# YannisLamp/crypto-recommendation

Measured on AMD Instinct MI355X. Metric: point hash+assign ops/sec at d=128, N=10M, K=256; 1/2/4/8 MI355X, higher is better.
Workload: dtype fp32 points; split-f16 MFMA scores (f32 accumulate); tuples, bucket IDs and cluster IDs bit-exact (x87-exact hashing, certified argmin); distances: certified f32, <= 2^-20 relative to the reference's fp64 (north star: 1e-5; the context's default LSHKM_DIST_CERTIFIED mode), LSHKM_DIST_EXACT for the r; 1 GPU; C3 Lloyd K=256 + C2 LSH L=5 k=4 hashing, N=10000000 per GPU, d=128; N_per_gpu=10000000, N_total=10000000, d=128, K=256, L=5, k=4, nb=100000, parallelism=dp1 (row shards)

## Files before the change

crypto-recommendation_amd/csrc/fused_hi.hip:

```cpp
#include "fused_impl.h"

namespace lshkm {

__host__ __device__ constexpr int fh_lds_bytes(int Kpad, bool hash) {
    return 16 + Kpad * FU_RS * 2 + Kpad * 4 + (hash ? 2 * 32 * FU_RS * 2 + FP_HC_BYTES : 0);
}
static_assert(fh_lds_bytes(FH_KMAX, true) <= 160 * 1024, "hi-only LDS image exceeds 160 KiB");
constexpr double FH_A = 130.0 * 0x1p-23;

constexpr int FH_WAVES_MPFAST = 12;
constexpr int FH_FAST_WAVES = 8;
template <bool HASH, bool MP, int MET, bool FAST = false>
__host__ __device__ constexpr int fh_waves() {
    return HASH && MP ? 12 : (MP && FAST ? FH_WAVES_MPFAST : (FAST && !MP ? FH_FAST_WAVES : 8));
}

__device__ inline int cosine_halves_finish(double sh0, double sl0, double ts0, double sh, double sl, double ts,
                                           double xa, double nbv, double& v) {
    const double mb = 2.0 * sqrt(__dmul_rn(xa, nbv)) * (1.0 + 0x1p-40);
    const double tsum = __dadd_rn(ts0, ts);
    if (!(tsum >= 0x1p-790)) return 2;
    IpAcc ip;
    const double t = __dadd_rn(sh0, sh);
    const double bb = __dsub_rn(t, sh0);
    const double e = __dadd_rn(__dsub_rn(sh0, __dsub_rn(t, bb)), __dsub_rn(sh, bb));
    ip.sh = t;
    ip.sl = __dadd_rn(__dadd_rn(sl0, sl), e);
    ip.ts = __dadd_rn(tsum * (1.0 + 0x1p-47), 0x1p-37 * mb);
    ip.mx = mb;
    double q, qr;
    const int st = ip.quot_status(__dmul_rn(sqrt(xa), sqrt(nbv)), q, qr);
    if (st == 0) v = __dsub_rn(1.0, q);
    return st;
}

__device__ inline int cosine_winner_halves(const float (&xf)[64], const double* __restrict__ crow_h, double nbv, int h,
                                           double& v) {
    double xa = 0.0;
#pragma unroll
    for (int s = 0; s < 8; s++) {
        if (h == 0) {
#pragma unroll
            for (int j = 0; j < 8; j++) {
                const double xj = (double)xf[8 * s + j];
                xa = __dadd_rn(xa, __dmul_rn(xj, xj));
            }
        }
        xa = take_from_lower(xa);
        if (h == 1) {
#pragma unroll
            for (int j = 0; j < 8; j++) {
                const double xj = (double)xf[8 * s + j];
                xa = __dadd_rn(xa, __dmul_rn(xj, xj));
            }
        }
        xa = take_from_upper(xa);
    }
    double sh = 0.0, sl = 0.0, ts = 0.0;
    double off = 0.0;
    double2 cb[4];
#pragma unroll
    for (int j = 0; j < 4; j++) cb[j] = *reinterpret_cast<const double2*>(crow_h + 2 * j);
#pragma unroll
    for (int s = 0; s < 8; s++) {
        double cv[8];
#pragma unroll
        for (int j = 0; j < 4; j++) { cv[2 * j] = cb[j].x; cv[2 * j + 1] = cb[j].y; }
        if (s + 1 < 8) {
#pragma unroll
            for (int j = 0; j < 4; j++) cb[j] = *reinterpret_cast<const double2*>(crow_h + 16 * (s + 1) + 2 * j);
        }
#pragma unroll
        for (int j = 0; j < 8; j++) {
            const double pj = __dmul_rn((double)xf[8 * s + j], cv[j]);
            const double t = __dadd_rn(sh, pj);
            const double bb = __dsub_rn(t, sh);
            const double e = __dadd_rn(__dsub_rn(sh, __dsub_rn(t, bb)), __dsub_rn(pj, bb));
            sh = t;
            sl = __dadd_rn(sl, e);
            ts = __dadd_rn(ts, fabs(__dadd_rn(t, off)));
        }
        const double other = swap_halves(sh, h);
        if (h == 1) ts = __dadd_rn(ts, 8.0 * fabs(__dsub_rn(other, off)));
        off = other;
    }
    const double sh0 = swap_halves(sh, h), sl0 = swap_halves(sl, h), ts0 = swap_halves(ts, h);
    if (h == 0) return 2;
    return cosine_halves_finish(sh0, sl0, ts0, sh, sl, ts, xa, nbv, v);
}

__device__ inline int cosine_winner_halves_x64(const FusedArgs& a, int64_t rowc, const double* __restrict__ crow_h,
                                               double nbv, int h, double& v) {
    double2 xn[4], xnn[4];
    load_x64_step(a, rowc, 0, h, xn);
    load_x64_step(a, rowc, 1, h, xnn);
    double sh = 0.0, sl = 0.0, ts = 0.0;
    double off = 0.0;
    double2 cb[4];
#pragma unroll
    for (int j = 0; j < 4; j++) cb[j] = *reinterpret_cast<const double2*>(crow_h + 2 * j);
#pragma unroll 1
    for (int s = 0; s < 8; s++) {
        double xv[8], cv[8];
#pragma unroll
        for (int j = 0; j < 4; j++) {
            xv[2 * j] = xn[j].x; xv[2 * j + 1] = xn[j].y;
            cv[2 * j] = cb[j].x; cv[2 * j + 1] = cb[j].y;
            xn[j] = xnn[j];
        }
        if (s + 2 < 8) load_x64_step(a, rowc, s + 2, h, xnn);
        if (s + 1 < 8) {
#pragma unroll
            for (int j = 0; j < 4; j++) cb[j] = *reinterpret_cast<const double2*>(crow_h + 16 * (s + 1) + 2 * j);
        }
#pragma unroll
        for (int j = 0; j < 8; j++) {
            const double pj = __dmul_rn(xv[j], cv[j]);
            const double t = __dadd_rn(sh, pj);
            const double bb = __dsub_rn(t, sh);
            const double e = __dadd_rn(__dsub_rn(sh, __dsub_rn(t, bb)), __dsub_rn(pj, bb));
            sh = t;
            sl = __dadd_rn(sl, e);
            ts = __dadd_rn(ts, fabs(__dadd_rn(t, off)));
        }
        const double other = swap_halves(sh, h);
        if (h == 1) ts = __dadd_rn(ts, 8.0 * fabs(__dsub_rn(other, off)));
        off = other;
    }
    const double sh0 = swap_halves(sh, h), sl0 = swap_halves(sl, h), ts0 = swap_halves(ts, h);
    if (h == 0) return 2;
    return cosine_halves_finish(sh0, sl0, ts0, sh, sl, ts, a.xn2[rowc], nbv, v);
}

constexpr int FH_GATH_STEP = 32 * 16 * 8;
constexpr int FH_GATH_WAVE = 2 * FH_GATH_STEP;
__host__ __device__ constexpr int fh_gath_off(int Kpad, bool hash) { return (fh_lds_bytes(Kpad, hash) + 255) & ~255; }
static_assert(fh_gath_off(FH_GATH_KMAX, true) + 8 * FH_GATH_WAVE <= 160 * 1024, "gather ring exceeds 160 KiB");

__device__ inline void glds16(const void* gsrc, uint32_t lds_dst) {
    unsigned keep;
    asm volatile("s_mov_b32 %0, m0\n\ts_mov_b32 m0, %2\n\ts_nop 0\n\tglobal_load_lds_dwordx4 %1, off\n\ts_mov_b32 m0, %0"
                 : "=&s"(keep) : "v"(gsrc), "s"(lds_dst) : "memory");
}

#ifndef LSHKM_ROWPF
#define LSHKM_ROWPF 3
#endif
constexpr int FH_ROWPF = LSHKM_ROWPF;
constexpr int FH_ROWPF_KMAX = 256;
constexpr int FH_ROWPF_WAVE = 32 * 64 * 4;
__host__ __device__ constexpr int fh_rowpf_off(int Kpad, bool hash) { return (fh_lds_bytes(Kpad, hash) + 255) & ~255; }
static_assert(fh_rowpf_off(FH_ROWPF_KMAX, true) + FH_FAST_WAVES * FH_ROWPF_WAVE <= 160 * 1024,
              "row prefetch buffers exceed 160 KiB");
static_assert(FH_ROWPF_KMAX <= FH_GATH_KMAX, "the FAST single-pass form runs where the gather ring would (fused.hip)");

__device__ inline void glds16s(const void* sbase, uint32_t voff, uint32_t lds_base, int lds_off) {
    unsigned keep;
    asm volatile("s_mov_b32 %0, m0\n\ts_add_u32 m0, %3, %4\n\ts_nop 0\n\tglobal_load_lds_dwordx4 %1, %2\n\ts_mov_b32 m0, %0"
                 : "=&s"(keep) : "v"(voff), "s"(sbase), "s"(lds_base), "n"(lds_off) : "memory", "scc");
}

template <bool HASH, bool MP = false, int MET = 0, int NIMG = 1, bool GATH = false, int ROWS = 0, bool FAST = false,
          int PF = 0>
__global__ __launch_bounds__((64 * fh_waves<HASH, MP, MET, FAST>()), 1) void fused_hi_kernel(FusedArgs a) {
    constexpr int FH_WAVES = fh_waves<HASH, MP, MET, FAST>();
    constexpr int FH_THREADS = 64 * FH_WAVES;
    static_assert(NIMG == 1 || (!MP && MET == 0), "two-image form: euclidean, single launch");
    static_assert(!GATH || (!MP && MET == 0 && NIMG == 1 && FH_WAVES == 8), "gather ring: euclidean single pass");
    static_assert(ROWS == 0 || (!HASH && !MP && NIMG == 1), "general rows: Lloyd without hashing, one pass");
    static_assert(!(GATH && ROWS == 2), "fp64 rows re-read x in the chain: register loads of the winner rows");
    static_assert(!FAST || (MET == 0 && ROWS != 2 && NIMG == 1 && !GATH), "fast distance: euclidean, fp32 rows");
    static_assert(PF == 0 || (FAST && !MP && ROWS == 0 && FH_WAVES == FH_FAST_WAVES), "row prefetch: the FAST single-pass form");
    constexpr bool PFR = (PF & 1) != 0, PFL = (PF & 2) != 0;
    extern __shared__ __attribute__((aligned(16))) char smem[];
    const int Kpad = a.Kpad;
    const bool fastd = FAST || a.fast_dist != 0;
    const int KI = NIMG == 2 ? FH_KMAX : Kpad;
    int* lcount = reinterpret_cast<int*>(smem);
    _Float16* lch = reinterpret_cast<_Float16*>(smem + 16);
    float* lcn = reinterpret_cast<float*>(lch + KI * FU_RS);
    _Float16* lvh = reinterpret_cast<_Float16*>(lcn + KI);
    _Float16* lvl = lvh + 32 * FU_RS;
    float* lpn0 = reinterpret_cast<float*>(lvl + 32 * FU_RS);
    float* lv10 = lpn0 + 32;
    float* lt0 = lv10 + 32;
    int32_t* lr0 = reinterpret_cast<int32_t*>(lt0 + 32);

    auto load_image = [&](int img) {
        const int r0 = img * KI, nr = NIMG == 2 && img == 1 ? Kpad - FH_KMAX : KI;
        constexpr int FH_CU = 8;
        for (int e0 = 0; e0 < nr * 16; e0 += FH_THREADS * FH_CU) {
            float4 v[FH_CU];
#pragma unroll
            for (int u = 0; u < FH_CU; u++) {
                const int e = e0 + u * FH_THREADS + (int)threadIdx.x < nr * 16 ? e0 + u * FH_THREADS + (int)threadIdx.x : 0;
                v[u] = *reinterpret_cast<const float4*>(a.Ch + (size_t)(r0 + (e >> 4)) * FU_D + (e & 15) * 8);
            }
#pragma unroll
            for (int u = 0; u < FH_CU; u++) {
                const int e = e0 + u * FH_THREADS + (int)threadIdx.x < nr * 16 ? e0 + u * FH_THREADS + (int)threadIdx.x : 0;
                *reinterpret_cast<float4*>(lch + (e >> 4) * FU_RS + (e & 15) * 8) = v[u];
            }
        }
        for (int e = threadIdx.x; e < nr; e += FH_THREADS) lcn[e] = a.cnh[r0 + e];
    };
    load_image(0);
    if (threadIdx.x < 3) lcount[threadIdx.x] = 0;
    int32_t* ambig_seg = a.ambig + (int64_t)blockIdx.x * a.seg_rows;
    unsigned long long* hfix_seg = a.hfix + (int64_t)blockIdx.x * a.seg_rows;
    unsigned long long* cfix_seg = a.cfix ? a.cfix + (int64_t)blockIdx.x * a.seg_rows : nullptr;
    if (HASH) {
        hash_stage_images<FH_THREADS>(a.Vh, a.Vl, lvh, lvl);
        if (threadIdx.x < 32) {
            const int f = threadIdx.x;
            const bool on = f < a.LK;
            float P = 0.f, Q = 0.f;
            if (on) hash_window<MET == 0>(a.pnorm[f], a.v1[f], MET == 0 ? a.tv[f] : 0.f, a.w, P, Q);
            lpn0[f] = P;
            lv10[f] = Q;
            lt0[f] = on && MET == 0 ? a.tv[f] : 0.f;
            lr0[f] = on && MET == 0 ? a.rv[f] : 0;
        }
    }
    __syncthreads();

    const int lane = threadIdx.x & 63;
    const int wave = PF != 0 ? __builtin_amdgcn_readfirstlane((int)(threadIdx.x >> 6)) : (int)(threadIdx.x >> 6);
    const int col = lane & 31, h = lane >> 5;
    const float cmaxf = a.cbound[3], crf = a.cbound[4], chf = a.cbound[5], cnf = a.cbound[6];
    const bool c_ok = __float_as_uint(a.cbound[2]) == 0u;
    const _Float16* my_h = lch + col * FU_RS + 8 * h;
    const int ntile32 = Kpad >> 5;
    const int64_t ntiles = (a.N + 31) >> 5;
    const double Ec = (0x1p-24 + FH_A) * (double)cnf + 0x1p-41 * (double)cmaxf * (double)cmaxf + 0x1p-18 * (double)cnf;

    const int64_t tstride = (int64_t)gridDim.x * FH_WAVES, tfirst = (int64_t)blockIdx.x * FH_WAVES;
    const int64_t nround = NIMG == 2 && ntiles > tfirst ? (ntiles - tfirst + tstride - 1) / tstride : 0;
    int64_t rd = 0;
    auto load_row = [&](int64_t tl, float (&dst)[64]) {
        const int64_t rr = tl * 32 + col, rc = rr < a.N ? rr : a.N - 1;
        if constexpr (ROWS != 0) load_row_gen<ROWS>(a, rc, h, dst);
        else load_row_b(a.X + rc * FU_D + 8 * h, dst);
    };
    auto load_half = [&](int64_t tl, int hf, float* dst) {
        const int64_t rr = tl * 32 + col, rc = rr < a.N ? rr : a.N - 1;
        const float* xr = a.X + rc * FU_D + 64 * hf + 8 * h;
#pragma unroll
        for (int s = 0; s < 4; s++) {
            const float4 p0 = *reinterpret_cast<const float4*>(xr + 16 * s);
            const float4 p1 = *reinterpret_cast<const float4*>(xr + 16 * s + 4);
            dst[8 * s + 0] = p0.x; dst[8 * s + 1] = p0.y; dst[8 * s + 2] = p0.z; dst[8 * s + 3] = p0.w;
            dst[8 * s + 4] = p1.x; dst[8 * s + 5] = p1.y; dst[8 * s + 6] = p1.z; dst[8 * s + 7] = p1.w;
        }
    };
    uint32_t pfbase = 0;
    if constexpr (PFL)
        pfbase = (uint32_t)__builtin_amdgcn_readfirstlane(
            (int)((uint32_t)(uintptr_t)(smem + fh_rowpf_off(Kpad, HASH)) + (uint32_t)wave * FH_ROWPF_WAVE));
    auto pf_dma = [&](int64_t tl) {
        const int64_t tls = ((int64_t)__builtin_amdgcn_readfirstlane((int)(tl >> 32)) << 32) |
                            (uint32_t)__builtin_amdgcn_readfirstlane((int)tl);
        const int64_t left = a.N - 1 - tls * 32;
        const int pmax = left < 31 ? (int)left : 31;
        const float* xt = a.X + tls * 32 * FU_D;
        if (pmax == 31) {
            const uint32_t w0 = (uint32_t)((lane >> 4) * (FU_D * 4) + 16 * ((lane & 15) ^ (lane >> 4)));
#pragma unroll
            for (int u = 0; u < 8; u++) glds16s(xt + u * 4 * FU_D, w0 ^ (uint32_t)(64 * (u & 3)), pfbase, u * 1024);
        } else {
#pragma unroll
            for (int u = 0; u < 8; u++) {
                const int p = 4 * u + (lane >> 4), pc = p < pmax ? p : pmax;
                glds16s(xt, (uint32_t)(pc * (FU_D * 4) + 16 * ((lane & 15) ^ (p & 15))), pfbase, u * 1024);
            }
        }
    };
    float xn[32];
    auto pf_next = [&](int64_t tl) {
        if constexpr (PF != 0) {
            if (tl + tstride < ntiles) {
                if constexpr (PFL) {
                    __builtin_amdgcn_s_waitcnt(0xC07F);
                    asm volatile("" ::: "memory");
                    pf_dma(tl + tstride);
                }
                if constexpr (PFR) load_half(tl + tstride, 1, xn);
            } else if constexpr (PFR) {
#pragma unroll
                for (int j = 0; j < 32; j++) xn[j] = 0.f;
            }
        }
    };
    if constexpr (PF != 0) {
        if (tfirst + wave < ntiles) {
            if constexpr (PFL) pf_dma(tfirst + wave);
            if constexpr (PFR) load_half(tfirst + wave, 1, xn);
            if constexpr (PFL) {
                __builtin_amdgcn_s_waitcnt(0x0F70);
                asm volatile("" ::: "memory");
            }
        }
    }
    PT_DECL
    for (int64_t tile = tfirst + wave; NIMG == 2 ? rd < nround : tile < ntiles; tile += tstride, rd++) {
        const int64_t row = tile * 32 + col;
        const bool valid = row < a.N;
        float xf[64];
        if constexpr (PF == 0) {
            load_row(tile, xf);
        } else {
            if constexpr (PFL) {
                if constexpr (!PFR) {
                    load_half(tile, 1, xf + 32);
                    asm volatile("" ::: "memory");
                }
                __builtin_amdgcn_s_waitcnt(PFR ? 0x4F70 : 0x0F78);
                asm volatile("" ::: "memory");
                const char* pb = smem + fh_rowpf_off(Kpad, HASH) + wave * FH_ROWPF_WAVE + col * 256;
#pragma unroll
                for (int c = 0; c < 8; c++) {
                    const float4 v = *reinterpret_cast<const float4*>(pb + 16 * ((4 * (c >> 1) + 2 * h + (c & 1)) ^ (col & 15)));
                    xf[4 * c] = v.x; xf[4 * c + 1] = v.y; xf[4 * c + 2] = v.z; xf[4 * c + 3] = v.w;
                }
            } else {
                load_half(tile, 0, xf);
            }
            if constexpr (PFR) {
#pragma unroll
                for (int j = 0; j < 32; j++) xf[32 + j] = xn[j];
            }
        }
        half8 bh[8];
        float2v n2a = {0.f, 0.f}, n2b = {0.f, 0.f}, r2 = {0.f, 0.f};
        double xn2, nx, nxr, nxh;
        bool x_ok;
        auto finish_norms = [&]() {
            float xn2f = (n2a.x + n2a.y) + (n2b.x + n2b.y);
            float xr2f = r2.x + r2.y;
            xn2f += __shfl_xor(xn2f, 32);
            xr2f += __shfl_xor(xr2f, 32);
            xn2 = (double)xn2f * (1.0 + 0x1p-16);
            nx = sqrt(xn2);
            nxr = sqrt((double)xr2f * (1.0 + 0x1p-16)) + 0x1p-100;
            if (ROWS == 2) nxr += 0x1p-24 * nx * (1.0 + 0x1p-20);
            nxh = nx + nxr;
            x_ok = xn2f <= FU_RANGE * FU_RANGE;
        };
        const bool hash_here = HASH;
        if (!hash_here) {
#pragma unroll
            for (int s = 0; s < 8; s++) {
                half8 unused;
                split_norm_step<false>(xf + 8 * s, bh[s], unused, n2a, n2b, r2);
            }
            pf_next(tile);
            finish_norms();
        }

        if (hash_here) {
            uint32_t fmask = 0;
            float acc_hi[16];
            {
                const _Float16* vh_row = lvh + col * FU_RS + 8 * h;
                const _Float16* vl_row = lvl + col * FU_RS + 8 * h;
                floatx16 tot;
#pragma unroll
                for (int s = 0; s < 8; s++) {
                    half8 bl;
                    split_norm_step<true>(xf + 8 * s, bh[s], bl, n2a, n2b, r2);
                    const floatx16 acc = hash_tile_step(s, vh_row, vl_row, bh[s], bl);
                    if (s == 0) {
                        tot = acc;
                    } else {
#pragma unroll
                        for (int r = 0; r < 16; r += 2) {
                            const float2v t2 = {tot[r], tot[r + 1]}, a2 = {acc[r], acc[r + 1]};
                            const float2v u2 = t2 + a2;
                            tot[r] = u2.x;
                            tot[r + 1] = u2.y;
                        }
                    }
                }
#pragma unroll
                for (int r = 0; r < 16; r++) acc_hi[r] = tot[r];
            }
            finish_norms();
            const float iw = MET == 1 ? 1.f : 1.0f / a.w;
            const float nxf = (float)nx * (1.f + 0x1p-20f);
            int hc = 0;
            asm volatile("" : "+v"(hc));
            const float* lt = lt0 + hc;
            const float* lP = lpn0 + hc;
            const float* lQ = lv10 + hc;
            const int32_t* lr = lr0 + hc;
            if (!x_ok && valid) fmask = (a.LK >= 32 ? 0xFFFFFFFFu : (1u << a.LK) - 1u);
#pragma unroll
            for (int g = 0; g < 4; g++) {
                const int l = 2 * g + h;
                if (l >= a.L || !valid) continue;
                const int64_t o = row * a.L + l;
                if constexpr (MET == 1) {
                    int gv = 0;
#pragma unroll
                    for (int q = 0; q < 4; q++) {
                        const int f = 4 * l + q;
                        int bit;
                        if (!certify_sign_f32(acc_hi[4 * g + q], nxf, lP[f], lQ[f], bit)) fmask |= 1u << f;
                        gv = (gv << 1) | bit;
                    }
                    if (a.phi) a.phi[o] = gv;
                    if (a.bucket) a.bucket[o] = gv;
                    continue;
                }
                int32_t hv[4];
#pragma unroll
                for (int q = 0; q < 4; q++) {
                    const int f = 4 * l + q;
                    if (!certify_floor_f32(acc_hi[4 * g + q], lt[f], iw, nxf, lP[f], lQ[f], hv[q])) fmask |= 1u << f;
                }
                if (a.tuples) *reinterpret_cast<int4*>(a.tuples + o * 4) = make_int4(hv[0], hv[1], hv[2], hv[3]);
                uint32_t hn = 0;
#pragma unroll
                for (int q = 0; q < 4; q++) hn += phi_term_small(hv[q], lr[4 * l + q]);
                const uint32_t ph = phi_final(hn);
                if (a.phi) a.phi[o] = (int32_t)ph;
                if (a.bucket) a.bucket[o] = bucket_fast(ph, a.bdiv);
            }
            fmask |= __shfl_xor(fmask, 32);
            const unsigned long long fb = __ballot(fmask != 0u && h == 1);
            if (fb) {
                const int leader = __builtin_ctzll(fb);
                int base = 0;
                if (lane == leader) base = atomicAdd(lcount + 1, __popcll(fb));
                base = __shfl(base, leader);
                if (fmask != 0u && h == 1)
                    hfix_seg[base + __popcll(fb & ((1ull << lane) - 1ull))] = ((unsigned long long)row << 32) | fmask;
            }
        }

        if (HASH) pf_next(tile);
        PT_MARK(0)
        const double E = (nxh * (double)crf + nxr * (double)cmaxf + FH_A * nxh * (double)chf + 0x1p-41 * xn2 +
                          0x1p-18 * nx * (double)cmaxf + (MET == 1 ? 0x1p-43 * nx : 0.0) + Ec) * (1.0 + 0x1p-20) +
                         1e-30;
        float m1 = -__builtin_inff(), m2 = -__builtin_inff();
        int t1 = 0;
        if (MP && !HASH && !a.pass_first) {
            const float4 st = a.part[tile * 64 + lane];
            m1 = st.x; m2 = st.y; t1 = __float_as_int(st.z);
        }
        const int tg0 = MP ? a.t0 : 0;
        __builtin_amdgcn_s_setprio(MFMA_PRIO);
        const int ntile_run = ntile32;
        auto run_tiles = [&](int ntl, int tgo) {
#pragma unroll 1
            for (int t = 0; t < ntl; t++) {
                const float m1_prev = m1;
                floatx16 acc;
                const float* cn_t = lcn + t * 32 + 4 * h;
#pragma unroll
                for (int g = 0; g < 4; g++) {
                    const float4 cn = *reinterpret_cast<const float4*>(cn_t + 8 * g);
                    acc[4 * g] = cn.x; acc[4 * g + 1] = cn.y; acc[4 * g + 2] = cn.z; acc[4 * g + 3] = cn.w;
                }
                const _Float16* arow = my_h + t * 32 * FU_RS;
#pragma unroll
                for (int s = 0; s < 8; s++) {
                    const half8 ah = *reinterpret_cast<const half8*>(arow + 16 * s);
                    acc = __builtin_amdgcn_mfma_f32_32x32x16_f16(ah, bh[s], acc, 0, 0, 0);
                }
                float sv[16];
#pragma unroll
                for (int r = 0; r < 16; r++) sv[r] = acc[r];
                tile_epilogue(sv, m1, m2);
                t1 = m1 != m1_prev ? t + tgo : t1;
            }
        };
        if (NIMG == 1) {
            run_tiles(ntile_run, tg0);
        } else {
            const int i0 = (int)(rd & 1);
            const int nA = FH_KMAX / 32, nB = (Kpad - FH_KMAX) / 32;
            run_tiles(i0 == 0 ? nA : nB, i0 * nA);
            __syncthreads();
            load_image(1 - i0);
            __syncthreads();
            run_tiles(i0 == 0 ? nB : nA, (1 - i0) * nA);
        }
        __builtin_amdgcn_s_setprio(0);
        PT_MARK(1)
        if (MP && (HASH || !a.pass_last)) {
            a.part[tile * 64 + lane] = make_float4(m1, m2, __int_as_float(t1), 0.f);
            continue;
        }
        const uint32_t l1 = __float_as_uint(m1) & 0xFu;
        const int i1 = t1 * 32 + 8 * (int)(l1 >> 2) + 4 * h + (int)(l1 & 3u);
        const float om1 = __shfl_xor(m1, 32), om2 = __shfl_xor(m2, 32);
        const int oi1 = __shfl_xor(i1, 32);
        const float M2 = fmaxf(fmaxf(m2, om2), fminf(m1, om1));
        const int I1 = (om1 > m1 || (om1 == m1 && oi1 < i1)) ? oi1 : i1;
        const float M1 = fmaxf(m1, om1);
        const double* crow = a.C64 + (size_t)I1 * FU_D + 8 * h;
        const char* gsrc[4];
        uint32_t gbase = 0;
        const bool g32 = GATH && a.C32 != nullptr && (__float_as_uint(a.cbound[7]) & 1u) == 0u;
        const int gstep = g32 ? 64 : 128;
        if (GATH && !fastd) {
            gbase = (uint32_t)__builtin_amdgcn_readfirstlane(
                (int)((uint32_t)(uintptr_t)(smem + fh_gath_off(Kpad, HASH)) + (uint32_t)wave * FH_GATH_WAVE));
            if (g32) {
#pragma unroll
                for (int u = 0; u < 2; u++) {
                    const int p = 16 * u + (lane >> 2);
                    const int Ip = __shfl(I1, p);
                    gsrc[u] = reinterpret_cast<const char*>(a.C32 + (size_t)Ip * FU_D + 4 * ((lane & 3) ^ ((p >> 2) & 3)));
                }
                gsrc[2] = gsrc[3] = gsrc[0];
#pragma unroll
                for (int s0 = 0; s0 < 2; s0++)
#pragma unroll
                    for (int u = 0; u < 2; u++) glds16(gsrc[u] + gstep * s0, gbase + s0 * FH_GATH_STEP + u * 1024);
            } else {
#pragma unroll
                for (int u = 0; u < 4; u++) {
                    const int p = 8 * u + (lane >> 3);
                    const int Ip = __shfl(I1, p);
                    gsrc[u] = reinterpret_cast<const char*>(a.C64 + (size_t)Ip * FU_D + 2 * ((lane & 7) ^ ((p >> 1) & 7)));
                }
#pragma unroll
                for (int s0 = 0; s0 < 2; s0++)
#pragma unroll
                    for (int u = 0; u < 4; u++) glds16(gsrc[u] + gstep * s0, gbase + s0 * FH_GATH_STEP + u * 1024);
            }
        }
        double2 gnext[4];
        float4 gnext32[2];
        auto gread = [&](int st) {
            const char* ring = smem + fh_gath_off(Kpad, HASH) + wave * FH_GATH_WAVE + (st & 1) * FH_GATH_STEP;
            if (g32) {
#pragma unroll
                for (int j = 0; j < 2; j++)
                    gnext32[j] = *reinterpret_cast<const float4*>(ring + (col >> 4) * 1024 + (col & 15) * 64 +
                                                                  16 * ((2 * h + j) ^ ((col >> 2) & 3)));
            } else {
#pragma unroll
                for (int j = 0; j < 4; j++)
                    gnext[j] = *reinterpret_cast<const double2*>(ring + col * 128 + 16 * ((4 * h + j) ^ ((col >> 1) & 7)));
            }
        };
        auto wait_step = [&]() {
            if (g32) __builtin_amdgcn_s_waitcnt(0x0F72);
            else __builtin_amdgcn_s_waitcnt(0x0F74);
        };
        auto ring_advance = [&](int s) {
            if (s + 2 < 8) {
                __builtin_amdgcn_s_waitcnt(0xC07F);
                asm volatile("" ::: "memory");
                if (g32) {
#pragma unroll
                    for (int u = 0; u < 2; u++) glds16(gsrc[u] + gstep * (s + 2), gbase + (s & 1) * FH_GATH_STEP + u * 1024);
                } else {
#pragma unroll
                    for (int u = 0; u < 4; u++) glds16(gsrc[u] + gstep * (s + 2), gbase + (s & 1) * FH_GATH_STEP + u * 1024);
                }
            }
            if (s + 1 < 8) {
                if (s + 2 < 8) wait_step();
                else __builtin_amdgcn_s_waitcnt(0x0F70);
                asm volatile("" ::: "memory");
                gread(s + 1);
            }
        };
        constexpr int XD = 4;
        double2 xring[XD][4];
        const int64_t rowc = row < a.N ? row : a.N - 1;
        if constexpr (ROWS == 2 && MET == 0) {
#pragma unroll
            for (int st = 0; st < XD; st++) load_x64_step(a, rowc, st, h, xring[st]);
        }
        double2 cbuf[4];
        if (MET == 0 && !GATH && !fastd) {
#pragma unroll
            for (int j = 0; j < 4; j++) cbuf[j] = *reinterpret_cast<const double2*>(crow + 2 * j);
        }
        const bool cert = x_ok && c_ok && ((double)M2 < (double)M1 - 2.0 * E);

        bool dok = true;
        double fdist = 0.0;
        if constexpr (MET == 0) {
            if (fastd) {
                const float* c32 = a.C32 + (size_t)I1 * FU_D + 8 * h;
                float2v q[4] = {};
                float4 cc[16];
                if constexpr (PF != 0) {
#pragma unroll
                    for (int s = 0; s < 8; s++) {
                        cc[2 * s] = *reinterpret_cast<const float4*>(c32 + 16 * s);
                        cc[2 * s + 1] = *reinterpret_cast<const float4*>(c32 + 16 * s + 4);
                    }
                    __builtin_amdgcn_sched_barrier(0);
                }
#pragma unroll
                for (int s = 0; s < 8; s++) {
                    float4 c0, c1;
                    if constexpr (PF != 0) {
                        c0 = cc[2 * s]; c1 = cc[2 * s + 1];
                    } else {
                        c0 = *reinterpret_cast<const float4*>(c32 + 16 * s);
                        c1 = *reinterpret_cast<const float4*>(c32 + 16 * s + 4);
                    }
                    const float2v cv[4] = {{c0.x, c0.y}, {c0.z, c0.w}, {c1.x, c1.y}, {c1.z, c1.w}};
#pragma unroll
                    for (int j = 0; j < 4; j++) {
                        const float2v xv = {xf[8 * s + 2 * j], xf[8 * s + 2 * j + 1]};
                        const float2v dv = xv - cv[j];
                        q[j] = __builtin_elementwise_fma(dv, dv, q[j]);
                    }
                }
                float t = ((q[0].x + q[0].y) + (q[1].x + q[1].y)) + ((q[2].x + q[2].y) + (q[3].x + q[3].y));
                t = t + swap_halves_f(t, h);
                const double S = (double)t, R = (double)a.rn32[I1];
                const double B = 14.2 * 0x1p-24 * S + 2.02 * R * sqrt(S) + 2.02 * R * R + 0x1p-100;
                dok = B <= 0x1p-19 * S;
                fdist = sqrt(S);
            }
        }
        const bool amb = valid && !(cert && dok);
        const unsigned long long amask = __ballot(amb && h == 1);
        if (amb && h == 1) {
            int base = 0;
            const int leader = __builtin_ctzll(amask);
            if (lane == leader) base = atomicAdd(lcount, __popcll(amask));
            base = __shfl(base, leader);
            ambig_seg[base + __popcll(amask & ((1ull << lane) - 1ull))] = (int32_t)row;
        }
        if constexpr (MET == 1) {
            bool fix = false;
            if (valid && cert) {
                double v = 0.0;
                int st;
                if constexpr (ROWS == 2) st = cosine_winner_halves_x64(a, row, a.C64 + (size_t)I1 * FU_D + 8 * h, a.nbv[I1], h, v);
                else st = cosine_winner_halves(xf, a.C64 + (size_t)I1 * FU_D + 8 * h, a.nbv[I1], h, v);
                if (h == 1) {
                    a.assign[row] = I1;
                    if (st == 0) a.dist[row] = v;
                    else fix = true;
                }
            }
            const unsigned long long fb = __ballot(fix);
            if (fb) {
                const int leader = __builtin_ctzll(fb);
                int base = 0;
                if (lane == leader) base = atomicAdd(lcount + 2, __popcll(fb));
                base = __shfl(base, leader);
                if (fix) cfix_seg[base + __popcll(fb & ((1ull << lane) - 1ull))] = (unsigned long long)row;
            }
        } else if (fastd) {
            if (h == 1 && valid && cert && dok) {
                a.assign[row] = I1;
                a.dist[row] = fdist;
            }
        } else {
            __builtin_amdgcn_s_setprio(CHAIN_PRIO);
            double acc = 0.0;
            PwAcc pw;
            double* pwl = nullptr;
            if constexpr (ROWS == 2) {
                if (a.pw_lds) pwl = reinterpret_cast<double*>(smem + a.pw_lds) + wave * 512;
            }
            if constexpr (GATH) {
                wait_step();
                asm volatile("" ::: "memory");
                gread(0);
            }
#pragma unroll
            for (int s = 0; s < 8; s++) {
                double sq[8];
                double2 cur[4];
                if constexpr (GATH) {
                    if (g32) {
#pragma unroll
                        for (int j = 0; j < 2; j++) {
                            cur[2 * j] = make_double2((double)gnext32[j].x, (double)gnext32[j].y);
                            cur[2 * j + 1] = make_double2((double)gnext32[j].z, (double)gnext32[j].w);
                        }
                    } else {
#pragma unroll
                        for (int j = 0; j < 4; j++) cur[j] = gnext[j];
                    }
                    ring_advance(s);
                } else {
#pragma unroll
                    for (int j = 0; j < 4; j++) cur[j] = cbuf[j];
                    if (s + 1 < 8) {
#pragma unroll
                        for (int j = 0; j < 4; j++) cbuf[j] = *reinterpret_cast<const double2*>(crow + 16 * (s + 1) + 2 * j);
                    }
                }
                double2 xcur[4];
                if constexpr (ROWS == 2) {
#pragma unroll
                    for (int j = 0; j < 4; j++) xcur[j] = xring[s % XD][j];
                    if (s + XD < 8) load_x64_step(a, rowc, s + XD, h, xring[s % XD]);
                } else {
#pragma unroll
                    for (int j = 0; j < 4; j++) xcur[j] = make_double2((double)xf[8 * s + 2 * j], (double)xf[8 * s + 2 * j + 1]);
                }
                double dv[8];
#pragma unroll
                for (int j = 0; j < 4; j++) {
                    const double2 cc = cur[j];
                    dv[2 * j] = __dsub_rn(xcur[j].x, cc.x);
                    dv[2 * j + 1] = __dsub_rn(xcur[j].y, cc.y);
                }
                if (ROWS == 2 && pwl) {
                    gp_sq_wave<8>(dv, sq, pwl);
                } else {
#pragma unroll
                    for (int j = 0; j < 8; j++) {
                        sq[j] = __dmul_rn(dv[j], dv[j]);
                        pw.add<ROWS == 2>(dv[j]);
                    }
                }
                if (h == 0) {
#pragma unroll
                    for (int j = 0; j < 8; j++) acc = __dadd_rn(acc, sq[j]);
                }
                acc = take_from_lower(acc);
                if (h == 1) {
#pragma unroll
                    for (int j = 0; j < 8; j++) acc = __dadd_rn(acc, sq[j]);
                }
                acc = take_from_upper(acc);
            }
            const bool pw_hard = pwl == nullptr && (pw.hard() || (ROWS != 2 && (__float_as_uint(a.cbound[7]) & 2u) != 0u));
            const int pw_other = __shfl_xor((int)pw_hard, 32);
            const bool hard = pw_hard || pw_other != 0;
            if (h == 1 && valid && cert) {
                a.assign[row] = I1;
                if (!hard) a.dist[row] = sqrt(acc);
            }
            const unsigned long long pb = __ballot(h == 1 && valid && cert && hard);
            if (pb) {
                const int leader = __builtin_ctzll(pb);
                int base = 0;
                if (lane == leader) base = atomicAdd(lcount + 2, __popcll(pb));
                base = __shfl(base, leader);
                if (h == 1 && valid && cert && hard) cfix_seg[base + __popcll(pb & ((1ull << lane) - 1ull))] = (unsigned long long)row;
            }
            __builtin_amdgcn_s_setprio(0);
        }
        PT_MARK(2)
    }
    PT_FLUSH
    __syncthreads();
    if (threadIdx.x < 2 && (!MP || (threadIdx.x == 0 ? (!HASH && a.pass_last != 0) : (HASH && a.pass_first)))) {
        const int c = lcount[threadIdx.x];
        a.seg_counts[SEG_SLOTS * blockIdx.x + threadIdx.x] = c;
        if (c) atomicAdd(threadIdx.x == 0 ? a.ambig_count : a.hfix_count, (unsigned long long)c);
    }
    if ((MET == 1 || !fastd) && threadIdx.x == 2 && (!MP || (!HASH && a.pass_last))) {
        const int c = lcount[2];
        a.cfix_counts[SEG_SLOTS * blockIdx.x + SEG_FIX] = c;
        if (c) atomicAdd(a.cfix_count, (unsigned long long)c);
    }
}

template <bool HASH, bool MP, int MET, int NIMG, bool GATH, int ROWS, bool FAST, int PF>
static void hi_launch(hipStream_t s, unsigned nblk, size_t lds, const FusedArgs& a) {
    hipLaunchKernelGGL((fused_hi_kernel<HASH, MP, MET, NIMG, GATH, ROWS, FAST, PF>), dim3(nblk),
                       dim3(64 * fh_waves<HASH, MP, MET, FAST>()), lds, s, a);
}

int launch_fused_hi_pass(hipStream_t s, unsigned nblk, const HiForm& f, FusedArgs a) {
    size_t lds = (size_t)fh_lds_bytes(f.two_image ? FH_KMAX : a.Kpad, f.hash);
    a.pw_lds = 0;
    if (f.gath) {
        if (a.Kpad > FH_GATH_KMAX) {
            set_error("launch_fused_hi_pass: the gather ring needs K <= 256");
            return -1;
        }
        lds = (size_t)fh_gath_off(a.Kpad, f.hash) + 8 * FH_GATH_WAVE;
    } else if (f.rows == 2 && f.metric == 0) {
        constexpr int PW_BYTES = fh_waves<false, false, 0>() * 512 * 8;
        const size_t off = (lds + 255) & ~(size_t)255;
        if (off + PW_BYTES <= 160 * 1024) {
            a.pw_lds = (int)off;
            lds = off + PW_BYTES;
        }
    }
    const int pf = f.rowpf ? FH_ROWPF : 0;
    if (pf != 0 && !(f.fast && !f.mp && f.rows == 0 && !f.gath && a.Kpad <= FH_ROWPF_KMAX)) {
        set_error("launch_fused_hi_pass: the row prefetch needs the fast single-pass form at K <= 256");
        return -1;
    }
    if (pf & 2) lds = (size_t)fh_rowpf_off(a.Kpad, f.hash) + FH_FAST_WAVES * FH_ROWPF_WAVE;
    const int nimg = f.two_image ? 2 : 1;
#define HI_CASE_PF(H, MP, MET, NIMG, GATH, ROWS, FAST, PF)                                                  \
    if (f.hash == (bool)H && f.mp == (bool)MP && f.metric == MET && nimg == NIMG && f.gath == (bool)GATH && \
        f.rows == ROWS && f.fast == (bool)FAST && pf == PF) {                                               \
        hi_launch<H, MP, MET, NIMG, GATH, ROWS, FAST, PF>(s, nblk, lds, a);                                 \
        return 0;                                                                                           \
    }
#define HI_CASE(H, MP, MET, NIMG, GATH, ROWS, FAST) HI_CASE_PF(H, MP, MET, NIMG, GATH, ROWS, FAST, 0)
    HI_CASE_PF(1, 0, 0, 1, 0, 0, 1, FH_ROWPF)
    HI_CASE_PF(0, 0, 0, 1, 0, 0, 1, FH_ROWPF)
    HI_CASE(1, 0, 0, 1, 0, 0, 1)
    HI_CASE(0, 0, 0, 1, 0, 0, 1)
    HI_CASE(1, 0, 0, 1, 1, 0, 0)
    HI_CASE(0, 0, 0, 1, 1, 0, 0)
    HI_CASE(1, 0, 0, 1, 0, 0, 0)
    HI_CASE(0, 0, 0, 1, 0, 0, 0)
    HI_CASE(1, 1, 0, 1, 0, 0, 0)
    HI_CASE(0, 1, 0, 1, 0, 0, 1)
    HI_CASE(0, 1, 0, 1, 0, 0, 0)
    HI_CASE(1, 0, 0, 2, 0, 0, 0)
    HI_CASE(0, 0, 0, 2, 0, 0, 0)
    HI_CASE(1, 0, 1, 1, 0, 0, 0)
    HI_CASE(0, 0, 1, 1, 0, 0, 0)
    HI_CASE(1, 1, 1, 1, 0, 0, 0)
    HI_CASE(0, 1, 1, 1, 0, 0, 0)
    HI_CASE(0, 0, 0, 1, 0, 1, 1)
    HI_CASE(0, 0, 0, 1, 1, 1, 0)
    HI_CASE(0, 0, 0, 1, 0, 1, 0)
    HI_CASE(0, 0, 1, 1, 0, 1, 0)
    HI_CASE(0, 0, 0, 1, 0, 2, 0)
    HI_CASE(0, 0, 1, 1, 0, 2, 0)
#undef HI_CASE
#undef HI_CASE_PF
    set_error("launch_fused_hi_pass: no kernel was built for this form");
    return -1;
}

}
```

crypto-recommendation_amd/csrc/hash_tile.h:

```cpp
#pragma once
#include "tile.h"

namespace lshkm {

template <int THREADS>
__device__ inline void hash_stage_images(const _Float16* __restrict__ Vh, const _Float16* __restrict__ Vl,
                                         _Float16* lvh, _Float16* lvl) {
    for (int e = threadIdx.x; e < 32 * 16; e += THREADS) {
        const int r = e >> 4, g = e & 15;
        *reinterpret_cast<float4*>(lvh + r * FU_RS + g * 8) = *reinterpret_cast<const float4*>(Vh + r * FU_D + g * 8);
        *reinterpret_cast<float4*>(lvl + r * FU_RS + g * 8) = *reinterpret_cast<const float4*>(Vl + r * FU_D + g * 8);
    }
}

template <bool EUCLID>
__device__ inline void hash_window(double pnorm, double v1, float t, float w, float& P, float& Q) {
    const double iwu = EUCLID ? (double)(1.0f / w) * (1.0 + 0x1p-20) : 1.0;
    const double tf = EUCLID ? fabs((double)t) : 0.0;
    P = (float)((FU_A1H * pnorm * (1.0 + 0x1p-20) + FU_A2 * FU_SQRT_D) * iwu * (1.0 + 0x1p-18));
    Q = (float)((FU_A2 * v1 * (1.0 + 0x1p-20) + (0x1p-40 + 0x1p-23) * tf) * iwu * (1.0 + 0x1p-18) + 0x1p-126);
}

__device__ inline void load_row_b(const float* __restrict__ xr, float (&dst)[64]) {
#pragma unroll
    for (int s = 0; s < 8; s++) {
        const float4 p0 = *reinterpret_cast<const float4*>(xr + 16 * s);
        const float4 p1 = *reinterpret_cast<const float4*>(xr + 16 * s + 4);
        dst[8 * s + 0] = p0.x; dst[8 * s + 1] = p0.y; dst[8 * s + 2] = p0.z; dst[8 * s + 3] = p0.w;
        dst[8 * s + 4] = p1.x; dst[8 * s + 5] = p1.y; dst[8 * s + 6] = p1.z; dst[8 * s + 7] = p1.w;
    }
}

template <bool LO>
__device__ __forceinline__ void split_norm_step(const float* x8, half8& hi, half8& lo, float2v& n2a, float2v& n2b,
                                                float2v& r2) {
    split8_hi<LO>(x8, hi, lo, r2);
#pragma unroll
    for (int j = 0; j < 8; j += 4) {
        const float2v u = {x8[j], x8[j + 1]}, v = {x8[j + 2], x8[j + 3]};
        n2a = __builtin_elementwise_fma(u, u, n2a);
        n2b = __builtin_elementwise_fma(v, v, n2b);
    }
}

__device__ __forceinline__ floatx16 hash_tile_step(int s, const _Float16* vh_row, const _Float16* vl_row,
                                                   const half8& bh, const half8& bl) {
    const half8 ah = *reinterpret_cast<const half8*>(vh_row + 16 * s);
    const half8 al = *reinterpret_cast<const half8*>(vl_row + 16 * s);
    const floatx16 z = {};
    floatx16 acc = __builtin_amdgcn_mfma_f32_32x32x16_f16(al, bh, z, 0, 0, 0);
    acc = __builtin_amdgcn_mfma_f32_32x32x16_f16(ah, bl, acc, 0, 0, 0);
    return __builtin_amdgcn_mfma_f32_32x32x16_f16(ah, bh, acc, 0, 0, 0);
}

__device__ __forceinline__ bool certify_floor_f32(float acc, float t, float iw, float nxf, float P, float Q, int32_t& v) {
    constexpr float G = (0x1p-22f + 0x1p-20f) * (1.f + 0x1p-18f);
    const float y = (acc + t) * iw;
    const float B = fmaf(fabsf(y), G, fmaf(nxf, P, Q));
    const float lo = floorf(y - B), hi = floorf(y + B);
    v = (int32_t)lo;
    return lo == hi;
}
__device__ __forceinline__ bool certify_sign_f32(float acc, float nxf, float P, float Q, int& bit) {
    const float B = fmaf(nxf, P, Q);
    bit = acc >= 0.f ? 1 : 0;
    return fabsf(acc) > B;
}

}
```

crypto-recommendation_amd/csrc/tile.h:

```cpp
#pragma once
#include <hip/hip_runtime.h>
#include <stdint.h>

namespace lshkm {

typedef _Float16 half8 __attribute__((ext_vector_type(8)));
typedef float floatx16 __attribute__((ext_vector_type(16)));

constexpr int FU_D = 128;
constexpr int FU_RS = FU_D + 8;

constexpr double FU_A1 = 1.25 * 0x1p-16;
constexpr double FU_A1H = 1.25 * 0x1p-18;
constexpr double FU_A2 = 0x1p-24;
constexpr float FU_RANGE = 32768.f;

struct BucketDiv {
    uint32_t m, nb;
    int sh, mode;
};
__host__ inline BucketDiv make_bucket_div(int64_t nb) {
    BucketDiv b{0u, 0u, 0, 0};
    if (nb <= 1) { b.mode = 1; return b; }
    if (nb >= (1ll << 31)) { b.mode = 2; return b; }
    int l = 0;
    while ((1ll << l) < nb) l++;
    b.m = (uint32_t)((((unsigned __int128)1 << (31 + l)) / (unsigned __int128)nb) + 1);
    b.nb = (uint32_t)nb;
    b.sh = l - 1;
    return b;
}

typedef float float2v __attribute__((ext_vector_type(2)));
constexpr double FU_SQRT_D = 11.313708498984761 * (1.0 + 0x1p-40);

typedef _Float16 half2v __attribute__((ext_vector_type(2)));
__device__ inline float resid_lo(float x, half2v hp) {
    float r;
    asm("v_fma_mix_f32 %0, %1, 1.0, -%2 op_sel_hi:[0,0,1]" : "=v"(r) : "v"(x), "v"(hp));
    return r;
}
__device__ inline float resid_hi(float x, half2v hp) {
    float r;
    asm("v_fma_mix_f32 %0, %1, 1.0, -%2 op_sel:[0,0,1] op_sel_hi:[0,0,1]" : "=v"(r) : "v"(x), "v"(hp));
    return r;
}

constexpr uint32_t PHI_M = 2147483647u;
__device__ inline uint32_t phi_term(int32_t h, int32_t r) {
    int64_t v = (int32_t)((uint32_t)h * (uint32_t)r);
    if (v >= (int64_t)PHI_M) v -= PHI_M;
    if (v < 0) v += PHI_M;
    if (v < 0) v += PHI_M;
    return (uint32_t)v;
}
__device__ inline uint32_t phi_final(uint32_t hn) {
    if (hn >= PHI_M) hn -= PHI_M;
    if (hn >= PHI_M) hn -= PHI_M;
    return hn;
}
__device__ inline uint32_t phi_term_small(int32_t h, int32_t r) {
    const int32_t p = __mul24(h, r);
    return p < 0 ? (uint32_t)p + PHI_M : (uint32_t)p;
}
__device__ inline int32_t bucket_fast(uint32_t ph, const BucketDiv& b) {
    if (b.mode == 1) return 0;
    if (b.mode == 2) return (int32_t)ph;
    const uint32_t q = __umulhi(ph, b.m) >> b.sh;
    return (int32_t)(ph - q * b.nb);
}

template <bool LO>
__device__ inline void split8_hi(const float* x, half8& hi, half8& lo, float2v& r2) {
#pragma unroll
    for (int j = 0; j < 8; j += 2) {
        const half2v hp = {(_Float16)x[j], (_Float16)x[j + 1]};
        hi[j] = hp.x;
        hi[j + 1] = hp.y;
        const float2v r = {resid_lo(x[j], hp), resid_hi(x[j + 1], hp)};
        r2 = __builtin_elementwise_fma(r, r, r2);
        if (LO) {
            lo[j] = (_Float16)r.x;
            lo[j + 1] = (_Float16)r.y;
        }
    }
}

}
```

Before: 5.066 billion point hash+assign ops/s.

## Ping-pong prefetch row registers, trim live hash groups, vectorize hash certification

Turns the tile loop into a lambda that is unrolled twice, so the prefetched upper half-row buffer alternates between two register arrays. This removes the per-tile copy of 32 floats from the prefetch buffer into the row. A new HG template parameter cuts the accumulated hash groups to 3 when L is 5 or 6, which reduces the MFMA result adds and the registers kept live. The per-function LDS loads for hash certification become float4 loads, and the phi sum is computed branch-free over four terms. The cost is a larger instantiated kernel and another template variant.

```diff
diff --git a/crypto-recommendation_amd/csrc/fused_hi.hip b/crypto-recommendation_amd/csrc/fused_hi.hip
--- a/crypto-recommendation_amd/csrc/fused_hi.hip
+++ b/crypto-recommendation_amd/csrc/fused_hi.hip
@@ -161,7 +161,7 @@
 }
 
 template <bool HASH, bool MP = false, int MET = 0, int NIMG = 1, bool GATH = false, int ROWS = 0, bool FAST = false,
-          int PF = 0>
+          int PF = 0, int HG = 4>
 __global__ __launch_bounds__((64 * fh_waves<HASH, MP, MET, FAST>()), 1) void fused_hi_kernel(FusedArgs a) {
     constexpr int FH_WAVES = fh_waves<HASH, MP, MET, FAST>();
     constexpr int FH_THREADS = 64 * FH_WAVES;
@@ -171,6 +171,7 @@
     static_assert(!(GATH && ROWS == 2), "fp64 rows re-read x in the chain: register loads of the winner rows");
     static_assert(!FAST || (MET == 0 && ROWS != 2 && NIMG == 1 && !GATH), "fast distance: euclidean, fp32 rows");
     static_assert(PF == 0 || (FAST && !MP && ROWS == 0 && FH_WAVES == FH_FAST_WAVES), "row prefetch: the FAST single-pass form");
+    static_assert(HG == 4 || (HASH && MET == 0 && PF != 0 && HG >= 1 && HG < 4), "fewer live hash groups: the prefetching FAST form");
     constexpr bool PFR = (PF & 1) != 0, PFL = (PF & 2) != 0;
     extern __shared__ __attribute__((aligned(16))) char smem[];
     const int Kpad = a.Kpad;
@@ -275,8 +276,8 @@
             }
         }
     };
-    float xn[32];
-    auto pf_next = [&](int64_t tl) {
+    float xua[32], xub[32];
+    auto pf_next = [&](int64_t tl, float (&xnx)[32]) {
         if constexpr (PF != 0) {
             if (tl + tstride < ntiles) {
                 if constexpr (PFL) {
@@ -284,17 +285,14 @@
                     asm volatile("" ::: "memory");
                     pf_dma(tl + tstride);
                 }
-                if constexpr (PFR) load_half(tl + tstride, 1, xn);
-            } else if constexpr (PFR) {
-#pragma unroll
-                for (int j = 0; j < 32; j++) xn[j] = 0.f;
+                if constexpr (PFR) load_half(tl + tstride, 1, xnx);
             }
         }
     };
     if constexpr (PF != 0) {
         if (tfirst + wave < ntiles) {
             if constexpr (PFL) pf_dma(tfirst + wave);
-            if constexpr (PFR) load_half(tfirst + wave, 1, xn);
+            if constexpr (PFR) load_half(tfirst + wave, 1, xua);
             if constexpr (PFL) {
                 __builtin_amdgcn_s_waitcnt(0x0F70);
                 asm volatile("" ::: "memory");
@@ -302,10 +300,12 @@
         }
     }
     PT_DECL
-    for (int64_t tile = tfirst + wave; NIMG == 2 ? rd < nround : tile < ntiles; tile += tstride, rd++) {
+    auto tile_body = [&](const int64_t tile, float (&xup)[32], float (&xnx)[32]) __attribute__((always_inline)) {
         const int64_t row = tile * 32 + col;
         const bool valid = row < a.N;
         float xf[64];
+        float* const xhi = PFR ? xup : xf + 32;
+        auto x8 = [&](int s) -> const float* { return s < 4 ? xf + 8 * s : xhi + 8 * (s - 4); };
         if constexpr (PF == 0) {
             load_row(tile, xf);
         } else {
@@ -324,10 +324,6 @@
                 }
             } else {
                 load_half(tile, 0, xf);
-            }
-            if constexpr (PFR) {
-#pragma unroll
-                for (int j = 0; j < 32; j++) xf[32 + j] = xn[j];
             }
         }
         half8 bh[8];
@@ -351,9 +347,9 @@
 #pragma unroll
             for (int s = 0; s < 8; s++) {
                 half8 unused;
-                split_norm_step<false>(xf + 8 * s, bh[s], unused, n2a, n2b, r2);
-            }
-            pf_next(tile);
+                split_norm_step<false>(x8(s), bh[s], unused, n2a, n2b, r2);
+            }
+            pf_next(tile, xnx);
             finish_norms();
         }
 
@@ -367,13 +363,13 @@
 #pragma unroll
                 for (int s = 0; s < 8; s++) {
                     half8 bl;
-                    split_norm_step<true>(xf + 8 * s, bh[s], bl, n2a, n2b, r2);
+                    split_norm_step<true>(x8(s), bh[s], bl, n2a, n2b, r2);
                     const floatx16 acc = hash_tile_step(s, vh_row, vl_row, bh[s], bl);
                     if (s == 0) {
                         tot = acc;
                     } else {
 #pragma unroll
-                        for (int r = 0; r < 16; r += 2) {
+                        for (int r = 0; r < 4 * HG; r += 2) {
                             const float2v t2 = {tot[r], tot[r + 1]}, a2 = {acc[r], acc[r + 1]};
                             const float2v u2 = t2 + a2;
                             tot[r] = u2.x;
@@ -389,13 +385,12 @@
             const float nxf = (float)nx * (1.f + 0x1p-20f);
             int hc = 0;
             asm volatile("" : "+v"(hc));
-            const float* lt = lt0 + hc;
             const float* lP = lpn0 + hc;
             const float* lQ = lv10 + hc;
-            const int32_t* lr = lr0 + hc;
+            const float* hb = lpn0 + hc + 4 * h;
             if (!x_ok && valid) fmask = (a.LK >= 32 ? 0xFFFFFFFFu : (1u << a.LK) - 1u);
 #pragma unroll
-            for (int g = 0; g < 4; g++) {
+            for (int g = 0; g < HG; g++) {
                 const int l = 2 * g + h;
                 if (l >= a.L || !valid) continue;
                 const int64_t o = row * a.L + l;
@@ -412,17 +407,15 @@
                     if (a.bucket) a.bucket[o] = gv;
                     continue;
                 }
+                const float4 P4 = *reinterpret_cast<const float4*>(hb + 8 * g);
+                const float4 Q4 = *reinterpret_cast<const float4*>(hb + 32 + 8 * g);
+                const float4 t4 = *reinterpret_cast<const float4*>(hb + 64 + 8 * g);
+                const int4 r4 = *reinterpret_cast<const int4*>(hb + 96 + 8 * g);
                 int32_t hv[4];
-#pragma unroll
-                for (int q = 0; q < 4; q++) {
-                    const int f = 4 * l + q;
-                    if (!certify_floor_f32(acc_hi[4 * g + q], lt[f], iw, nxf, lP[f], lQ[f], hv[q])) fmask |= 1u << f;
-                }
+                fmask |= certify_floor4_f32(acc_hi + 4 * g, t4, iw, nxf, P4, Q4, hv) << (4 * l);
                 if (a.tuples) *reinterpret_cast<int4*>(a.tuples + o * 4) = make_int4(hv[0], hv[1], hv[2], hv[3]);
-                uint32_t hn = 0;
-#pragma unroll
-                for (int q = 0; q < 4; q++) hn += phi_term_small(hv[q], lr[4 * l + q]);
-                const uint32_t ph = phi_final(hn);
+                const int32_t rv4[4] = {r4.x, r4.y, r4.z, r4.w};
+                const uint32_t ph = phi_final(phi_sum4_small(hv, rv4));
                 if (a.phi) a.phi[o] = (int32_t)ph;
                 if (a.bucket) a.bucket[o] = bucket_fast(ph, a.bdiv);
             }
@@ -438,7 +431,7 @@
             }
         }
 
-        if (HASH) pf_next(tile);
+        if (HASH) pf_next(tile, xnx);
         PT_MARK(0)
         const double E = (nxh * (double)crf + nxr * (double)cmaxf + FH_A * nxh * (double)chf + 0x1p-41 * xn2 +
                           0x1p-18 * nx * (double)cmaxf + (MET == 1 ? 0x1p-43 * nx : 0.0) + Ec) * (1.0 + 0x1p-20) +
@@ -491,7 +484,7 @@
         PT_MARK(1)
         if (MP && (HASH || !a.pass_last)) {
             a.part[tile * 64 + lane] = make_float4(m1, m2, __int_as_float(t1), 0.f);
-            continue;
+            return;
         }
         const uint32_t l1 = __float_as_uint(m1) & 0xFu;
         const int i1 = t1 * 32 + 8 * (int)(l1 >> 2) + 4 * h + (int)(l1 & 3u);
@@ -612,7 +605,7 @@
                     const float2v cv[4] = {{c0.x, c0.y}, {c0.z, c0.w}, {c1.x, c1.y}, {c1.z, c1.w}};
 #pragma unroll
                     for (int j = 0; j < 4; j++) {
-                        const float2v xv = {xf[8 * s + 2 * j], xf[8 * s + 2 * j + 1]};
+                        const float2v xv = {x8(s)[2 * j], x8(s)[2 * j + 1]};
                         const float2v dv = xv - cv[j];
                         q[j] = __builtin_elementwise_fma(dv, dv, q[j]);
                     }
@@ -704,7 +697,7 @@
                     if (s + XD < 8) load_x64_step(a, rowc, s + XD, h, xring[s % XD]);
                 } else {
 #pragma unroll
-                    for (int j = 0; j < 4; j++) xcur[j] = make_double2((double)xf[8 * s + 2 * j], (double)xf[8 * s + 2 * j + 1]);
+                    for (int j = 0; j < 4; j++) xcur[j] = make_double2((double)x8(s)[2 * j], (double)x8(s)[2 * j + 1]);
                 }
                 double dv[8];
 #pragma unroll
@@ -751,6 +744,16 @@
             __builtin_amdgcn_s_setprio(0);
         }
         PT_MARK(2)
+    };
+    if constexpr (PFR) {
+        for (int64_t tile = tfirst + wave; tile < ntiles; tile += 2 * tstride) {
+            tile_body(tile, xua, xub);
+            if (tile + tstride >= ntiles) break;
+            tile_body(tile + tstride, xub, xua);
+        }
+    } else {
+        for (int64_t tile = tfirst + wave; NIMG == 2 ? rd < nround : tile < ntiles; tile += tstride, rd++)
+            tile_body(tile, xua, xub);
     }
     PT_FLUSH
     __syncthreads();
@@ -766,9 +769,9 @@
     }
 }
 
-template <bool HASH, bool MP, int MET, int NIMG, bool GATH, int ROWS, bool FAST, int PF>
+template <bool HASH, bool MP, int MET, int NIMG, bool GATH, int ROWS, bool FAST, int PF, int HG>
 static void hi_launch(hipStream_t s, unsigned nblk, size_t lds, const FusedArgs& a) {
-    hipLaunchKernelGGL((fused_hi_kernel<HASH, MP, MET, NIMG, GATH, ROWS, FAST, PF>), dim3(nblk),
+    hipLaunchKernelGGL((fused_hi_kernel<HASH, MP, MET, NIMG, GATH, ROWS, FAST, PF, HG>), dim3(nblk),
                        dim3(64 * fh_waves<HASH, MP, MET, FAST>()), lds, s, a);
 }
 
@@ -796,13 +799,18 @@
     }
     if (pf & 2) lds = (size_t)fh_rowpf_off(a.Kpad, f.hash) + FH_FAST_WAVES * FH_ROWPF_WAVE;
     const int nimg = f.two_image ? 2 : 1;
-#define HI_CASE_PF(H, MP, MET, NIMG, GATH, ROWS, FAST, PF)                                                  \
+    const int hg = f.hash && pf != 0 && (a.L == 5 || a.L == 6) ? 3 : 4;
+#define HI_CASE_HG(H, MP, MET, NIMG, GATH, ROWS, FAST, PF, HG)                                              \
     if (f.hash == (bool)H && f.mp == (bool)MP && f.metric == MET && nimg == NIMG && f.gath == (bool)GATH && \
-        f.rows == ROWS && f.fast == (bool)FAST && pf == PF) {                                               \
-        hi_launch<H, MP, MET, NIMG, GATH, ROWS, FAST, PF>(s, nblk, lds, a);                                 \
+        f.rows == ROWS && f.fast == (bool)FAST && pf == PF && hg == HG) {                                   \
+        hi_launch<H, MP, MET, NIMG, GATH, ROWS, FAST, PF, HG>(s, nblk, lds, a);                             \
         return 0;                                                                                           \
     }
+#define HI_CASE_PF(H, MP, MET, NIMG, GATH, ROWS, FAST, PF) HI_CASE_HG(H, MP, MET, NIMG, GATH, ROWS, FAST, PF, 4)
 #define HI_CASE(H, MP, MET, NIMG, GATH, ROWS, FAST) HI_CASE_PF(H, MP, MET, NIMG, GATH, ROWS, FAST, 0)
+#if LSHKM_ROWPF != 0
+    HI_CASE_HG(1, 0, 0, 1, 0, 0, 1, FH_ROWPF, 3)
+#endif
     HI_CASE_PF(1, 0, 0, 1, 0, 0, 1, FH_ROWPF)
     HI_CASE_PF(0, 0, 0, 1, 0, 0, 1, FH_ROWPF)
     HI_CASE(1, 0, 0, 1, 0, 0, 1)
@@ -827,6 +835,7 @@
     HI_CASE(0, 0, 0, 1, 0, 2, 0)
     HI_CASE(0, 0, 1, 1, 0, 2, 0)
 #undef HI_CASE
+#undef HI_CASE_HG
 #undef HI_CASE_PF
     set_error("launch_fused_hi_pass: no kernel was built for this form");
     return -1;
diff --git a/crypto-recommendation_amd/csrc/hash_tile.h b/crypto-recommendation_amd/csrc/hash_tile.h
--- a/crypto-recommendation_amd/csrc/hash_tile.h
+++ b/crypto-recommendation_amd/csrc/hash_tile.h
@@ -61,6 +61,15 @@
     v = (int32_t)lo;
     return lo == hi;
 }
+__device__ __forceinline__ uint32_t certify_floor4_f32(const float* acc4, const float4& t4, float iw, float nxf,
+                                                       const float4& P4, const float4& Q4, int32_t (&v)[4]) {
+    const float t[4] = {t4.x, t4.y, t4.z, t4.w}, P[4] = {P4.x, P4.y, P4.z, P4.w}, Q[4] = {Q4.x, Q4.y, Q4.z, Q4.w};
+    uint32_t bad = 0;
+#pragma unroll
+    for (int q = 0; q < 4; q++)
+        if (!certify_floor_f32(acc4[q], t[q], iw, nxf, P[q], Q[q], v[q])) bad |= 1u << q;
+    return bad;
+}
 __device__ __forceinline__ bool certify_sign_f32(float acc, float nxf, float P, float Q, int& bit) {
     const float B = fmaf(nxf, P, Q);
     bit = acc >= 0.f ? 1 : 0;
diff --git a/crypto-recommendation_amd/csrc/tile.h b/crypto-recommendation_amd/csrc/tile.h
--- a/crypto-recommendation_amd/csrc/tile.h
+++ b/crypto-recommendation_amd/csrc/tile.h
@@ -63,6 +63,12 @@
     const int32_t p = __mul24(h, r);
     return p < 0 ? (uint32_t)p + PHI_M : (uint32_t)p;
 }
+__device__ inline uint32_t phi_sum4_small(const int32_t (&h)[4], const int32_t (&r)[4]) {
+    const int32_t p0 = __mul24(h[0], r[0]), p1 = __mul24(h[1], r[1]), p2 = __mul24(h[2], r[2]), p3 = __mul24(h[3], r[3]);
+    const uint32_t sp = (uint32_t)p0 + (uint32_t)p1 + (uint32_t)p2 + (uint32_t)p3;
+    const uint32_t ss = (uint32_t)((p0 >> 31) + (p1 >> 31) + (p2 >> 31) + (p3 >> 31));
+    return sp + ss - (ss << 31);
+}
 __device__ inline int32_t bucket_fast(uint32_t ph, const BucketDiv& b) {
     if (b.mode == 1) return 0;
     if (b.mode == 2) return (int32_t)ph;
```

New measurement: 5.161 billion point hash+assign ops/s (median of 6 runs). 1.02x the previous value.
